# Algy/fast-slic

Measured on AMD Instinct MI355X. Metric: megapixels/sec @10 iters (1280x720 & 4K, K=1600); % HBM roofline, higher is better.
Workload: dtype u8/u16/i32 (integer SLIC); 1 GPU; 1280x720 RGB, K=1600, 10 iters (configs[1]), 8 frames/GPU; frames_per_gpu=8, global_frames=8, slots_per_gpu=6, submissions_per_launch_group=up to 2 (dynamic batching of the pipeline), inputs=device-resident uint8 RGB, device int16 labels, parallelism=frames sharded across GPUs, no collective

## Files before the change

### fast_slic_amd/_binding.py

```python
import ctypes as C
import os
import subprocess
import threading

import numpy as np

ARCH_NAME = "hip/gfx950"
_HERE = os.path.dirname(os.path.abspath(__file__))
_LIB_PATH = os.path.join(_HERE, "libfslic_hip.so")

CLUSTER_DTYPE = np.dtype([
    ("y", "<f4"), ("x", "<f4"), ("r", "<f4"), ("g", "<f4"), ("b", "<f4"), ("a", "<f4"),
    ("number", "<u2"), ("is_active", "u1"), ("is_updatable", "u1"), ("num_members", "<u4"),
])
assert CLUSTER_DTYPE.itemsize == 32

FSLIC_OK, FSLIC_E_INVALID, FSLIC_E_UNSUPPORTED, FSLIC_E_HIP, FSLIC_E_INTERNAL = range(5)


class Params(C.Structure):
    _fields_ = [
        ("max_iter", C.c_int32), ("compactness", C.c_float), ("min_size_factor", C.c_float),
        ("subsample_stride", C.c_int32), ("convert_to_lab", C.c_int32),
        ("manhattan_spatial_dist", C.c_int32), ("preemptive", C.c_int32),
        ("preemptive_thres", C.c_float), ("num_threads", C.c_int32), ("debug_mode", C.c_int32),
        ("abi", C.c_int32), ("variant", C.c_int32), ("reserved", C.c_int32 * 4),
    ]


EXPORTS = [
    "fslic_hip_device_count", "fslic_hip_create", "fslic_hip_destroy", "fslic_hip_initialize_clusters",
    "fslic_hip_iterate", "fslic_hip_iterate_device", "fslic_hip_iterate_batch", "fslic_hip_submit_group",
    "fslic_hip_wait_group", "fslic_hip_rgb_to_lab",
    "fslic_hip_enforce_connectivity", "fslic_hip_last_prelabels", "fslic_hip_last_timing_report",
    "fslic_hip_last_device_times", "fslic_hip_set_launch_timing", "fslic_hip_last_assign_loop", "fslic_hip_last_group_frames", "fslic_hip_last_path", "fslic_hip_last_launch_mode", "fslic_hip_group_done", "fslic_hip_last_error", "fslic_hip_version",
    "fslic_hip_get_connectivity", "fslic_hip_knn_connectivity", "fslic_hip_get_mask_density", "fslic_hip_cluster_density_to_mask",
    "fslic_hip_pipeline_submit", "fslic_hip_pipeline_drain", "fslic_hip_pipeline_batching", "fslic_hip_last_host_topk_frames",
    "fslic_hip_separate_pass_redos", "fslic_hip_copy_bandwidth", "fslic_hip_last_recorder_report",
    "fslic_hip_crf_new", "fslic_hip_crf_free", "fslic_hip_crf_copy", "fslic_hip_crf_get_params", "fslic_hip_crf_set_params",
    "fslic_hip_crf_set_compat", "fslic_hip_crf_get_compat", "fslic_hip_crf_num_classes", "fslic_hip_crf_first_time",
    "fslic_hip_crf_last_time", "fslic_hip_crf_num_frames", "fslic_hip_crf_pop_frame", "fslic_hip_crf_push_frame", "fslic_hip_crf_frame",
    "fslic_hip_crf_frame_time", "fslic_hip_crf_frame_set_clusters", "fslic_hip_crf_frame_get_clusters",
    "fslic_hip_crf_frame_set_connectivity", "fslic_hip_crf_frame_set_connectivity_csr", "fslic_hip_crf_frame_get_connectivity",
    "fslic_hip_crf_frame_set_mask", "fslic_hip_crf_frame_set_proba", "fslic_hip_crf_frame_set_unbiased", "fslic_hip_crf_frame_set_unary",
    "fslic_hip_crf_frame_get_unary", "fslic_hip_crf_frame_spatial_energy", "fslic_hip_crf_frame_temporal_energy",
    "fslic_hip_crf_frame_get_inferred", "fslic_hip_crf_frame_reset_inferred", "fslic_hip_crf_initialize", "fslic_hip_crf_inference",
    "fslic_hip_crf_expf_host", "fslic_hip_crf_expf_device",
    "fslic_hip_pool_workspace_size", "fslic_hip_pool", "fslic_hip_pool_finalize", "fslic_hip_unpool",
]

_lib = None
_lib_lock = threading.Lock()


def build_library(force=False):
    csrc = os.path.join(_HERE, "csrc")
    args = ["make", "-s", "-C", csrc]
    if force:
        args.append("-B")
    subprocess.check_call(args)
    return _LIB_PATH


def _preload_torch_hip_runtime():
    import importlib.util
    import sys
    if "torch" in sys.modules:
        return
    try:
        spec = importlib.util.find_spec("torch")
    except (ImportError, ValueError):
        spec = None
    if spec is None or not spec.origin:
        return
    cand = os.path.join(os.path.dirname(spec.origin), "lib", "libamdhip64.so")
    if os.path.exists(cand):
        try:
            C.CDLL(cand, mode=C.RTLD_GLOBAL)
        except OSError:
            pass


def load_library():
    global _lib
    with _lib_lock:
        if _lib is not None:
            return _lib
        _preload_torch_hip_runtime()
        if not os.path.exists(_LIB_PATH):
            raise ImportError(
                "fast_slic_amd: %s is missing; build it with `python -c 'import __graft_entry__ as g; g.build()'` "
                "or `make -C fast_slic_amd/csrc` (there is no CPU fallback)" % _LIB_PATH)
        lib = C.CDLL(os.environ.get("FSLIC_LIB") or _LIB_PATH)
        vp, i32 = C.c_void_p, C.c_int
        lib.fslic_hip_device_count.restype = i32
        lib.fslic_hip_create.argtypes = [i32, i32, C.POINTER(vp)]
        lib.fslic_hip_destroy.argtypes = [vp]
        lib.fslic_hip_destroy.restype = None
        lib.fslic_hip_initialize_clusters.argtypes = [i32, i32, i32, vp, vp]
        lib.fslic_hip_iterate.argtypes = [vp, C.POINTER(Params), i32, i32, i32, vp, vp, vp]
        lib.fslic_hip_iterate_device.argtypes = [vp, i32, C.POINTER(Params), i32, i32, i32, vp, vp, vp]
        lib.fslic_hip_iterate_batch.argtypes = [vp, C.POINTER(Params), i32, i32, i32, i32, vp, vp, vp, i32]
        lib.fslic_hip_submit_group.argtypes = [vp, i32, C.POINTER(Params), i32, i32, i32, i32, vp, vp, vp]
        lib.fslic_hip_wait_group.argtypes = [vp, i32]
        lib.fslic_hip_pipeline_submit.argtypes = [vp, C.POINTER(Params), i32, i32, i32, i32, vp, vp, vp]
        lib.fslic_hip_pipeline_drain.argtypes = [vp, C.POINTER(C.c_double), C.POINTER(C.c_longlong), C.POINTER(C.c_longlong), C.POINTER(C.c_longlong)]
        lib.fslic_hip_pipeline_batching.argtypes = [vp, i32]
        lib.fslic_hip_last_host_topk_frames.argtypes = [vp, i32]
        lib.fslic_hip_separate_pass_redos.argtypes = [vp, i32]
        if hasattr(lib, "fslic_hip_copy_bandwidth"):
            lib.fslic_hip_copy_bandwidth.argtypes = [vp, C.c_size_t, i32, C.POINTER(C.c_double)]
        lib.fslic_hip_group_done.argtypes = [vp, i32]
        lib.fslic_hip_rgb_to_lab.argtypes = [vp, i32, i32, vp, i32, vp]
        lib.fslic_hip_enforce_connectivity.argtypes = [vp, vp, i32, i32, i32, i32]
        lib.fslic_hip_last_prelabels.argtypes = [vp, i32, vp]
        lib.fslic_hip_last_timing_report.argtypes = [vp]
        lib.fslic_hip_last_timing_report.restype = C.c_char_p
        if hasattr(lib, "fslic_hip_last_recorder_report"):
            lib.fslic_hip_last_recorder_report.argtypes = [vp, C.POINTER(C.c_char_p), C.POINTER(C.c_size_t)]
        lib.fslic_hip_last_device_times.argtypes = [vp, i32, C.POINTER(C.c_float), C.POINTER(C.c_float)]
        lib.fslic_hip_set_launch_timing.argtypes = [vp, i32]
        lib.fslic_hip_last_assign_loop.argtypes = [vp, i32, C.POINTER(C.c_float), C.POINTER(C.c_double), C.POINTER(C.c_int)]
        lib.fslic_hip_last_group_frames.argtypes = [vp, i32]
        lib.fslic_hip_last_path.argtypes = [vp, i32]
        lib.fslic_hip_last_launch_mode.argtypes = [vp, i32]
        if hasattr(lib, "fslic_hip_lab_force_generic"):
            lib.fslic_hip_lab_force_generic.argtypes = [vp, i32]
        lib.fslic_hip_last_error.restype = C.c_char_p
        lib.fslic_hip_version.restype = C.c_char_p
        lib.fslic_hip_get_connectivity.argtypes = [vp, i32, i32, i32, vp, vp, vp]
        lib.fslic_hip_knn_connectivity.argtypes = [i32, i32, i32, vp, C.c_size_t, vp, vp]
        lib.fslic_hip_get_mask_density.argtypes = [vp, i32, i32, i32, vp, vp, vp, vp]
        lib.fslic_hip_cluster_density_to_mask.argtypes = [vp, i32, i32, i32, vp, vp, vp]
        if hasattr(lib, "fslic_hip_crf_new"):
            _declare_crf(lib)
        if hasattr(lib, "fslic_hip_pool"):
            _declare_pool(lib)
        _lib = lib
        return lib


def _declare_crf(lib):
    vp, i32, sz, f32 = C.c_void_p, C.c_int, C.c_size_t, C.c_float
    for name, args in [
        ("new", [sz, sz, C.POINTER(vp)]), ("copy", [vp, C.POINTER(vp)]), ("get_params", [vp, vp]), ("set_params", [vp, vp]),
        ("set_compat", [vp, i32, f32]), ("get_compat", [vp, i32, C.POINTER(f32)]), ("num_classes", [vp, C.POINTER(sz), C.POINTER(sz)]),
        ("first_time", [vp]), ("last_time", [vp]), ("pop_frame", [vp]), ("push_frame", [vp, C.POINTER(vp)]),
        ("frame", [vp, i32, C.POINTER(vp)]), ("frame_time", [vp]), ("frame_set_clusters", [vp, vp]), ("frame_get_clusters", [vp, vp]),
        ("frame_set_connectivity", [vp, i32, vp, vp, sz]), ("frame_set_connectivity_csr", [vp, i32, vp, vp]),
        ("frame_get_connectivity", [vp, vp, vp]), ("frame_set_mask", [vp, vp, f32]), ("frame_set_proba", [vp, vp]),
        ("frame_set_unbiased", [vp]), ("frame_set_unary", [vp, vp]), ("frame_get_unary", [vp, vp]),
        ("frame_spatial_energy", [vp, i32, i32, C.POINTER(f32)]), ("frame_temporal_energy", [vp, vp, i32, C.POINTER(f32)]),
        ("frame_get_inferred", [vp, vp]), ("frame_reset_inferred", [vp]), ("initialize", [vp]), ("inference", [vp, vp, sz]),
        ("expf_host", [vp, vp, sz, i32]), ("expf_device", [vp, vp, vp, sz]),
    ]:
        f = getattr(lib, "fslic_hip_crf_" + name)
        f.argtypes = args
        f.restype = i32
    lib.fslic_hip_crf_free.argtypes = [vp]
    lib.fslic_hip_crf_free.restype = None
    lib.fslic_hip_crf_num_frames.argtypes = [vp]
    lib.fslic_hip_crf_num_frames.restype = sz


def _declare_pool(lib):
    vp, i32 = C.c_void_p, C.c_int
    lib.fslic_hip_pool_workspace_size.argtypes = [i32, i32, i32, i32, C.POINTER(C.c_size_t)]
# ... 3 lines not shown
    for name in ("pool_workspace_size", "pool", "pool_finalize", "unpool"):
        getattr(lib, "fslic_hip_" + name).restype = i32


def _raise(rc):
    msg = load_library().fslic_hip_last_error().decode("utf-8", "replace")
    if rc == FSLIC_E_INVALID:
        raise ValueError(msg)
    if rc == FSLIC_E_UNSUPPORTED:
        raise NotImplementedError(msg)
    raise RuntimeError(msg)


def _check(rc):
    if rc != FSLIC_OK:
        _raise(rc)


class Engine(object):

    def __init__(self, device=0, n_slots=1):
        lib = load_library()
        h = C.c_void_p()
        _check(lib.fslic_hip_create(int(device), int(n_slots), C.byref(h)))
        self._h = h
        self.device = int(device)
        self.n_slots = int(n_slots)

    def close(self):
        if getattr(self, "_h", None):
            load_library().fslic_hip_destroy(self._h)
            self._h = None

    def __del__(self):
        try:
            self.close()
        except Exception:
            pass

    def rgb_to_lab(self, image, convert=True):
        image = np.ascontiguousarray(image, dtype=np.uint8)
        H, W, ch = image.shape
        if ch != 3:
            raise ValueError("nchan != 3")
        out = np.empty((H, W, 4), np.uint8)
        _check(load_library().fslic_hip_rgb_to_lab(self._h, H, W, image.ctypes.data, int(bool(convert)), out.ctypes.data))
        return out

    def enforce_connectivity(self, labels_u16, K, min_threshold):
        out = np.ascontiguousarray(labels_u16, dtype=np.uint16).copy()
        H, W = out.shape
        _check(load_library().fslic_hip_enforce_connectivity(self._h, out.ctypes.data, H, W, int(K), int(min_threshold)))
        return out

    @staticmethod
    def _plane(a, dtype):
        if isinstance(a, (int, np.integer)):
            return C.c_void_p(int(a)), None
        arr = np.ascontiguousarray(a, dtype=dtype)
        return C.c_void_p(arr.ctypes.data), arr

    def get_connectivity(self, labels, H, W, K):
        ptr, keep = self._plane(labels, np.uint16)
        num = np.zeros(K, np.int32)
        nb = np.zeros((K, 12), np.uint32)
        _check(load_library().fslic_hip_get_connectivity(self._h, H, W, int(K), ptr, num.ctypes.data, nb.ctypes.data))
        return num, nb

    def get_mask_density(self, clusters, labels, mask, H, W):
        lp, k1 = self._plane(labels, np.uint16)
        mp, k2 = self._plane(mask, np.uint8)
        cl = np.ascontiguousarray(clusters)
        dens = np.zeros(cl.shape[0], np.uint8)
        _check(load_library().fslic_hip_get_mask_density(self._h, H, W, cl.shape[0], cl.ctypes.data, lp, mp, dens.ctypes.data))
        return dens

    def cluster_density_to_mask(self, labels, densities, H, W, out=None):
        lp, k1 = self._plane(labels, np.uint16)
        d = np.ascontiguousarray(densities, dtype=np.uint8)
        if out is None:
            res = np.empty((H, W), np.uint8)
            op = C.c_void_p(res.ctypes.data)
        else:
            res, op = out, C.c_void_p(int(out))
        _check(load_library().fslic_hip_cluster_density_to_mask(self._h, H, W, d.shape[0], lp, d.ctypes.data, op))
        return res

    def iterate(self, image, clusters, params):
        H, W, _ = image.shape
        labels = np.empty((H, W), np.uint16)
        _check(load_library().fslic_hip_iterate(self._h, C.byref(params), H, W, clusters.shape[0],
                                                image.ctypes.data, clusters.ctypes.data, labels.ctypes.data))
        return labels

    def iterate_device(self, d_rgb_ptr, d_labels_ptr, H, W, clusters, params, slot=0):
        _check(load_library().fslic_hip_iterate_device(self._h, int(slot), C.byref(params), H, W, clusters.shape[0],
                                                       C.c_void_p(d_rgb_ptr), clusters.ctypes.data, C.c_void_p(d_labels_ptr)))

    def iterate_batch(self, rgb_ptrs, cluster_arrays, label_ptrs, H, W, params, device_ptrs):
        n = len(rgb_ptrs)
        K = cluster_arrays[0].shape[0]
        PA = C.c_void_p * n
        a_rgb = PA(*[C.c_void_p(int(p)) for p in rgb_ptrs])
        a_cl = PA(*[C.c_void_p(c.ctypes.data) for c in cluster_arrays])
        a_lab = PA(*[C.c_void_p(int(p)) for p in label_ptrs])
        _check(load_library().fslic_hip_iterate_batch(self._h, C.byref(params), H, W, K, n,
# ... 315 lines not shown
```

### fast_slic_amd/csrc/cca.hip

```cpp
#include "device_common.h"

namespace fslic {

constexpr uint32_t kNoAdopt = 0xFFFFFFFFu;
static __device__ __forceinline__ uint32_t* n_parent(const CcaDev& c, uint32_t n) { return reinterpret_cast<uint32_t*>(c.nrec + n); }
static __device__ __forceinline__ uint32_t n_leader(const CcaDev& c, uint32_t n) { return reinterpret_cast<const uint32_t*>(c.nrec + n)[1]; }
static __device__ __forceinline__ uint32_t n_local(const CcaDev& c, uint32_t n) { return reinterpret_cast<const uint32_t*>(c.nrec + n)[2]; }
static __device__ __forceinline__ uint32_t n_adopt(const CcaDev& c, uint32_t n) { return reinterpret_cast<const uint32_t*>(c.nrec + n)[3]; }

static __device__ __forceinline__ uint32_t lds_ld(uint32_t* p) {
    return __hip_atomic_load(p, __ATOMIC_RELAXED, __HIP_MEMORY_SCOPE_WORKGROUP);
}
static __device__ __forceinline__ void lds_st(uint32_t* p, uint32_t v) {
    __hip_atomic_store(p, v, __ATOMIC_RELAXED, __HIP_MEMORY_SCOPE_WORKGROUP);
}
static __device__ __forceinline__ uint32_t lds_find(uint32_t* par, uint32_t x) {
    for (;;) {
        const uint32_t p = lds_ld(par + x);
        if (p == x) return x;
        const uint32_t gp = lds_ld(par + p);
        if (gp == p) return p;
        lds_st(par + x, gp);
        x = gp;
    }
// ... 6 lines not shown
        if (a < b) { const uint32_t t = a; a = b; b = t; }
        const uint32_t old = atomicMin(par + a, b);
        if (old == a) return;
        a = old;
    }
}

static __device__ __forceinline__ uint32_t lds_find_ro(uint32_t* par, uint32_t x) {
    uint32_t p = lds_ld(par + x);
    while (p != x) { x = p; p = lds_ld(par + x); }
    return x;
}

typedef unsigned long long u64;
static __device__ __forceinline__ uint32_t lane_left0(uint32_t v) { return (uint32_t)__builtin_amdgcn_update_dpp(0, (int)v, 0x138 , 0xF, 0xF, true); }
static __device__ __forceinline__ uint32_t lane_left_or(uint32_t old, uint32_t v) { return (uint32_t)__builtin_amdgcn_update_dpp((int)old, (int)v, 0x138, 0xF, 0xF, false); }
static __device__ __forceinline__ uint32_t rank_in(u64 m) { return __builtin_amdgcn_mbcnt_hi((uint32_t)(m >> 32), __builtin_amdgcn_mbcnt_lo((uint32_t)m, 0u)); }
static __device__ __forceinline__ uint32_t* lds_at(uint32_t* base, uint32_t off) { return reinterpret_cast<uint32_t*>(reinterpret_cast<char*>(base) + off); }
static __device__ __forceinline__ void ldsb_union(uint32_t* par, uint32_t a, uint32_t b) {
    for (;;) {
        for (;;) {
            const uint32_t pa = lds_ld(lds_at(par, a)), pb = lds_ld(lds_at(par, b));
            if (pa == a && pb == b) break;
            a = pa; b = pb;
        }
        if (a == b) return;
        if (a < b) { const uint32_t t = a; a = b; b = t; }
        const uint32_t old = atomicMin(lds_at(par, a), b);
        if (old == a) return;
        a = old;
    }
}

#if defined(FSLIC_LAB) && FSLIC_LAB == 2
#define LOC_STAMP(i_) do { __syncthreads(); if (threadIdx.x == 0) c.cand_leader[(size_t)c.N - 8 * (size_t)(blockIdx.z * gridDim.y + blockIdx.y + 1) + (i_)] = (int32_t)((uint32_t)__builtin_amdgcn_s_memrealtime() - loc_t); } while (0)
#else
#define LOC_STAMP(i_) do { } while (0)
#endif
__global__ __launch_bounds__(256) __attribute__((amdgpu_num_sgpr(80))) void k_cca_local(CcaDev c) {
    const int tile_x = (int)blockIdx.y, tile_y = (int)blockIdx.z;
    c.select((int)blockIdx.x);
#if defined(FSLIC_LAB) && FSLIC_LAB == 2
    const uint32_t loc_t = (uint32_t)__builtin_amdgcn_s_memrealtime();
    if (threadIdx.x == 0) c.cand_leader[(size_t)c.N - 8 * (size_t)(blockIdx.z * gridDim.y + blockIdx.y + 1) + 7] = (int32_t)loc_t;
#endif
    constexpr int T = kCcaTile;
    constexpr int TH = kCcaTileH;
    constexpr int RW = TH / 4;
    static_assert(T == 64 && RW == 8, "lane = column, eight rows per wavefront");
    __shared__ uint32_t s_last[4][T];
    __shared__ uint32_t s_par[T * TH];
    __shared__ uint32_t s_area[T * TH];
    __shared__ uint32_t s_nroots, s_base;
    if (threadIdx.x == 0) s_nroots = 0;
    const int lane = LANE();
    const int wave = (int)rfl((uint32_t)(threadIdx.x >> 6));
    const int tx0 = tile_x * T, ty0 = tile_y * TH;
    const int ly0 = wave * RW;
    const int ncols = min(c.W - tx0, T), nrows = min(max(c.H - (ty0 + ly0), 0), RW);
    const u64 colmask = ncols >= 64 ? ~0ull : ((1ull << ncols) - 1ull);
#define ROW_MASK(i_) ((i_) < nrows ? colmask : 0ull)

    const uint16_t* const rowp = c.in + ((size_t)(ty0 + ly0) * c.W + tx0);
    uint32_t lbl[RW];
#pragma unroll
    for (int i = 0; i < RW; ++i) {
        lbl[i] = 0x10000u | (uint32_t)((i & 1) << 6) | (uint32_t)lane;
        if (lanes(ROW_MASK(i))) lbl[i] = (uint32_t)rowp[(size_t)i * c.W + lane];
    }
    LOC_STAMP(0);
    uint32_t nodev[RW];
    uint32_t up_root = 0, pend_a = 0, pend_b = 0;
    u64 pending = 0;
    auto run_pending = [&]() {
#if !(FSLIC_EXP & 128)
        if (lanes(pending)) ldsb_union(s_par, pend_a, pend_b);
#endif
        pending = 0;
    };
#pragma unroll
    for (int i = 0; i < RW; ++i) {
        const uint32_t l = lbl[i];
        const u64 m = ballot(l != lane_left0(l)) | 1ull;
        const uint32_t node = ((uint32_t)(ly0 + i) << 8) + (rank_in(m >> 1) << 2);
        nodev[i] = node;
        if (lanes(m)) { *lds_at(s_par, node) = node; *lds_at(s_area, node) = 0u; }
        if (i == RW - 1) s_last[wave][lane] = l | (node << 17);
        uint32_t cur_root = node;
        if (i > 0) {
            const u64 same = ballot(lbl[i - 1] == l);
            const u64 other = ballot(lane_left0(up_root) != up_root);
            const u64 rep = same & (m | other | ~(same << 1));
#if !(FSLIC_EXP & 64)
            if (lanes(rep)) __hip_atomic_fetch_min(lds_at(s_par, node), up_root, __ATOMIC_RELAXED, __HIP_MEMORY_SCOPE_WORKGROUP);
            cur_root = lds_ld(lds_at(s_par, node));
#endif
            const u64 need = rep & ballot(up_root != cur_root);
            if (need & pending) run_pending();
            const bool nd = lanes(need);
            pend_a = nd ? up_root : pend_a;
            pend_b = nd ? cur_root : pend_b;
            pending |= need;
        }
        up_root = cur_root;
    }
    run_pending();
    lds_barrier();
    LOC_STAMP(1);
    if (wave > 0) {
        const uint32_t l = lbl[0];
        const uint32_t prev = s_last[wave - 1][lane];
        const u64 m = ballot(l != lane_left0(l)) | 1ull;
        const u64 same = ballot((prev & 0x1FFFFu) == l);
        const u64 first = same & (m | ~(same << 1));
#if !(FSLIC_EXP & 128)
        if (lanes(first)) ldsb_union(s_par, nodev[0], prev >> 17);
#endif
    }
    lds_barrier();
    LOC_STAMP(2);
    uint32_t root[RW];
#pragma unroll
    for (int i = 0; i < RW; ++i) root[i] = lds_ld(lds_at(s_par, nodev[i]));
#pragma unroll
    for (int i = 0; i < RW; ++i) root[i] = lds_ld(lds_at(s_par, root[i]));
    for (;;) {
        uint32_t nx[RW];
#pragma unroll
        for (int i = 0; i < RW; ++i) nx[i] = lds_ld(lds_at(s_par, root[i]));
        u64 moved = 0;
#pragma unroll
        for (int i = 0; i < RW; ++i) { moved |= ballot(nx[i] != root[i]); root[i] = nx[i]; }
        if (!moved) break;
    }
    uint32_t pos[RW];
    uint32_t wcount = 0;
    const uint32_t lane_p1 = (uint32_t)lane + 1u;
#pragma unroll
    for (int i = 0; i < RW; ++i) {
        const u64 ok = ROW_MASK(i);
        const uint32_t l = lbl[i];
        const u64 m = ballot(l != lane_left0(l)) | 1ull;
        const u64 e = (m >> 1) | (1ull << 63);
        const uint32_t len_part = (lanes(e) ? lane_p1 : 0u) - (lanes(m) ? (uint32_t)lane : 0u);
#if !(FSLIC_EXP & 512)
        if (lanes((m | e) & ok)) atomicAdd(lds_at(s_area, root[i]), len_part);
#endif
        const u64 mr = m & ok & ballot(root[i] == nodev[i]);
        pos[i] = lanes(mr) ? wcount + rank_in(mr) : 0xFFFFFFFFu;
        wcount += (uint32_t)__popcll(mr);
    }
    LOC_STAMP(3);
    uint32_t wbase = 0;
    if (wcount != 0u && lanes(1ull)) {
        asm volatile("ds_add_rtn_u32 %0, %1, %2\n\ts_waitcnt lgkmcnt(0)" : "=v"(wbase) : "v"((uint32_t)(size_t)(__attribute__((address_space(3))) uint32_t*)&s_nroots), "v"(wcount) : "memory");
    }
    wbase = rfl(wbase);
    lds_barrier();
    LOC_STAMP(4);
    if (wave == 0 && lanes(1ull)) {
        const uint32_t nr = lds_ld(&s_nroots);
        uint32_t base = 0;
        if (nr) asm volatile("global_atomic_add %0, %1, %2, off sc0\n\ts_waitcnt vmcnt(0)" : "=v"(base) : "v"(c.counters), "v"(nr) : "memory");
        lds_st(&s_base, base);
    }
#pragma unroll
    for (int i = 0; i < RW; ++i)
        if (pos[i] != 0xFFFFFFFFu) lds_st(lds_at(s_par, root[i]), wbase + pos[i]);
    lds_barrier();
    LOC_STAMP(5);
    const uint32_t nbase = (uint32_t)(tile_y * (int)gridDim.y + tile_x) * (uint32_t)kCcaTilePx;
    const uint32_t gbase = s_base + wbase;
    uint32_t ar[RW];
#pragma unroll
    for (int i = 0; i < RW; ++i) ar[i] = lds_ld(lds_at(s_area, root[i]));
    wave_lds_sync();
    uint32_t* const stage = s_area + ly0 * T;
    uint32_t* const s_edge = &s_last[wave][lane ? 1 : 0];
    const __amdgpu_buffer_rsrc_t lr = __builtin_amdgcn_make_buffer_rsrc(c.lid, 0, (int)((uint32_t)c.N * 2u), 0x00020000);
    uint32_t up_id = 0xFFFu;
#pragma unroll
    for (int i = 0; i < RW; ++i) {
        const uint32_t y = (uint32_t)(ty0 + ly0 + i);
        const uint32_t id = lds_ld(lds_at(s_par, root[i]));
        const uint32_t left_id = lane_left_or(tile_x == 0 ? up_id : 0xFFFu, id);
        if (lanes(ROW_MASK(i))) __builtin_amdgcn_raw_buffer_store_b16((uint16_t)id, lr, lane * 2, (int)((y * (uint32_t)c.W + (uint32_t)tx0) * 2u), 16 );
        if (lanes(0x8000000000000001ull)) lds_st(s_edge + 2 * i, lbl[i] | (id << 16));
        if (pos[i] != 0xFFFFFFFFu) lds_st(stage + pos[i], (uint32_t)(i * T + lane) | ((ar[i] - 1u) << 9) | (left_id << 20));
        up_id = id;
    }
    wave_lds_sync();
    const uint32_t n0 = nbase + wbase;
    const uint32_t first_px = (uint32_t)(ty0 + ly0) * (uint32_t)c.W + (uint32_t)tx0;
    for (uint32_t j = (uint32_t)lane; j < wcount; j += 64u) {
        const uint32_t w = lds_ld(stage + j);
        const uint32_t n = n0 + j, a = ((w >> 9) & 0x7FFu) + 1u, ad = w >> 20;
        c.nrec[n] = make_uint4(n, first_px + __umul24((w >> 6) & 7u, (uint32_t)c.W) + (w & 63u), a, ad == 0xFFFu ? kNoAdopt : nbase + ad);
        c.narea[n] = a;
        c.roots[gbase + j] = n;
    }
    if (lane < 2 * RW) (c.vedge + (size_t)(nbase / (uint32_t)kCcaTilePx) * (2 * TH))[2 * ly0 + lane] = lds_ld(&s_last[wave][lane]);
    LOC_STAMP(6);
#undef ROW_MASK
}

static __device__ __forceinline__ uint32_t g_load(uint32_t* p) {
    return __hip_atomic_load(p, __ATOMIC_RELAXED, __HIP_MEMORY_SCOPE_AGENT);
}
static __device__ __forceinline__ uint32_t node_at(const CcaDev& c, int y, int x, size_t p) {
    return (uint32_t)((y / kCcaTileH) * c.tiles_x + x / kCcaTile) * (uint32_t)kCcaTilePx + (uint32_t)c.lid[p];
}
static __device__ __forceinline__ uint32_t node_of(const CcaDev& c, uint32_t p) {
    const int y = (int)(p / (uint32_t)c.W);
    return node_at(c, y, (int)(p - (uint32_t)y * (uint32_t)c.W), p);
}
static __device__ __forceinline__ uint32_t g_find(const CcaDev& c, uint32_t x) {
    for (;;) {
        const uint32_t p = g_load(n_parent(c, x));
        if (p == x) return x;
        const uint32_t gp = g_load(n_parent(c, p));
        if (gp == p) return p;
        __hip_atomic_store(n_parent(c, x), gp, __ATOMIC_RELAXED, __HIP_MEMORY_SCOPE_AGENT);
        x = gp;
    }
}
static __device__ __forceinline__ void g_union(const CcaDev& c, uint32_t a, uint32_t b) {
    for (;;) {
        a = g_find(c, a);
        b = g_find(c, b);
        if (a == b) return;
        if (n_leader(c, a) < n_leader(c, b)) { const uint32_t t = a; a = b; b = t; }
        if (atomicCAS(n_parent(c, a), a, b) == a) return;
    }
}

static __device__ __forceinline__ uint2 g_load2(const CcaDev& c, uint32_t n) {
    const unsigned long long v = __hip_atomic_load(reinterpret_cast<unsigned long long*>(c.nrec + n), __ATOMIC_RELAXED, __HIP_MEMORY_SCOPE_AGENT);
    return make_uint2((uint32_t)v, (uint32_t)(v >> 32));
}
static __device__ __forceinline__ uint32_t g_find_leader(const CcaDev& c, uint32_t& x, uint2 r) {
    for (;;) {
// ... 484 lines not shown
                return;
            }
            tie_heap_select(c, M, (uint32_t)K, astar, s_area, s_lead, s_key, s_bcnt, s_bstart, s_bfill, s_w);
            if (tid == 0) c.counters[3] = 0u;
            return;
        }
    }
    int bsh = 0;
    while ((((uint32_t)c.N - 1u) >> bsh) >= (uint32_t)kSelBuckets) bsh++;
    for (int i = tid; i < 3 * kSelBuckets; i += 1024) s_bcnt[i] = 0;
    __syncthreads();
    for (uint32_t i = tid; i < M; i += 1024)
        if (s_area[i] >= astar) atomicAdd(&s_bcnt[s_lead[i] >> bsh], 1u);
    __syncthreads();
    {
        const uint32_t a = s_bcnt[2 * tid], b = s_bcnt[2 * tid + 1];
        uint32_t n_keep;
        const uint32_t ex = block_excl_scan_1024(a + b, s_w, n_keep);
        s_bstart[2 * tid] = ex;
        s_bstart[2 * tid + 1] = ex + a;
    }
    __syncthreads();
    for (uint32_t i = tid; i < M; i += 1024)
        if (s_area[i] >= astar) {
            const uint32_t b = s_lead[i] >> bsh;
            s_key[s_bstart[b] + atomicAdd(&s_bfill[b], 1u)] = s_lead[i];
        }
    __syncthreads();
    for (uint32_t i0 = tid; i0 < M; i0 += 4096) {
        uint32_t me[4], r[4], nd[4];
        bool kept[4];
#pragma unroll
        for (int u = 0; u < 4; ++u) nd[u] = c.cand_area[min(i0 + 1024u * u, M - 1u)];
#pragma unroll
        for (int u = 0; u < 4; ++u) {
            const uint32_t i = i0 + 1024u * u;
            kept[u] = i < M && s_area[i] >= astar;
            me[u] = kept[u] ? s_lead[i] : 0u;
            r[u] = 0u;
            if (kept[u]) {
                const uint32_t b = me[u] >> bsh;
                const uint32_t lo = s_bstart[b], hi = lo + s_bcnt[b];
                r[u] = lo;
                for (uint32_t j = lo; j < hi; ++j) r[u] += (uint32_t)(s_key[j] < me[u]);
            }
        }
#pragma unroll
        for (int u = 0; u < 4; ++u) if (kept[u]) c.nfinal[nd[u]] = (uint16_t)r[u];
    }
    if (tid == 0) c.counters[3] = 0u;
}

static int root_pass_blocks(const CcaDev& c) {
    const int b = (c.N / 12 + 255) / 256;
    return b < 1 ? 1 : b;
}

void launch_cca_phase1(const CcaDev& c, int nframes, hipStream_t st) {
    constexpr int T = kCcaTile;
    const int tx = (c.W + T - 1) / T, ty = (c.H + kCcaTileH - 1) / kCcaTileH;
    launch(k_cca_local, dim3(nframes, tx, ty), dim3(256), 0, st, c);
    const int nh = (ty - 1) * ((c.W + kSeamPx - 1) / kSeamPx), nv = (tx - 1) * ((c.H + kSeamPx - 1) / kSeamPx);
    if (nh + nv > 0)
        launch(k_cca_border, dim3((nh + nv + 255) / 256, nframes), dim3(256), 0, st, c, nh, nv);
    launch(k_cca_compress, dim3(root_pass_blocks(c) * nframes), dim3(256), 0, st, c, nframes);
}

void launch_cca_select(const CcaDev& c, int nframes, hipStream_t st) {
    long long need = (long long)c.N / (c.min_threshold > 1 ? c.min_threshold : 1) + 1;
    int cap = 1024;
    while (cap < need && cap < kSelCap) cap <<= 1;
    if (cap > kSelCap) cap = kSelCap;
    const size_t lds = (3 * (size_t)cap + 3 * (size_t)kSelBuckets) * sizeof(uint32_t);
    static_assert(kSelBins <= 3 * kSelBuckets, "the selection histogram reuses the ranking buckets");
    static std::atomic<int> attr_state[64];
    if (!max_dynamic_lds_on_this_device(k_cca_select, (int)((3 * (size_t)kSelCap + 3 * (size_t)kSelBuckets) * sizeof(uint32_t)), attr_state)) {
        while (cap > 1024 && (3 * (size_t)cap + 3 * (size_t)kSelBuckets) * sizeof(uint32_t) > 64 * 1024) cap >>= 1;
        const size_t lds_small = (3 * (size_t)cap + 3 * (size_t)kSelBuckets) * sizeof(uint32_t);
        launch(k_cca_select, dim3(nframes), dim3(1024), lds_small, st, c, cap);
        return;
    }
    launch(k_cca_select, dim3(nframes), dim3(1024), lds, st, c, cap);
}

__global__ __launch_bounds__(256) void k_cca_reset_final(CcaDev c) {
    const uint32_t n = c.counters[0];
    for (uint32_t i = blockIdx.x * blockDim.x + threadIdx.x; i < n; i += gridDim.x * blockDim.x) {
        const uint32_t r = c.roots[i];
        if (*n_parent(c, r) == r) c.nfinal[r] = 0xFFFFu;
    }
}
__global__ void k_cca_set_kept(CcaDev c, const int32_t* __restrict__ leaders, const uint16_t* __restrict__ labels, int n) {
    const int i = blockIdx.x * blockDim.x + threadIdx.x;
    if (i < n) c.nfinal[node_of(c, (uint32_t)leaders[i])] = labels[i];
}
__global__ void k_cca_gather_area(CcaDev c) {
    const uint32_t M = c.counters[1];
    for (uint32_t i = blockIdx.x * blockDim.x + threadIdx.x; i < M; i += gridDim.x * blockDim.x) c.cand_area[i] = c.narea[node_of(c, (uint32_t)c.cand_leader[i])];
}
void launch_cca_gather_area(const CcaDev& c, hipStream_t st) {
    launch(k_cca_gather_area, dim3(64), dim3(256), 0, st, c);
}

void launch_cca_set_kept(const CcaDev& c, const int32_t* d_leaders, const uint16_t* d_labels, int n, hipStream_t st) {
    launch(k_cca_reset_final, dim3(root_pass_blocks(c)), dim3(256), 0, st, c);
    if (n <= 0) return;
    launch(k_cca_set_kept, dim3((n + 255) / 256), dim3(256), 0, st, c, d_leaders, d_labels, n);
// ... 124 lines not shown
```

### fast_slic_amd/csrc/host_utils.cpp

```cpp
#include "engine_internal.h"

#include <algorithm>
#include <cmath>
#include <cstring>

using namespace fslic;

extern "C" {

int fslic_hip_initialize_clusters(int H, int W, int K, const uint8_t* rgb, fslic_cluster* cl) {
    if (!rgb || !cl) return fail(FSLIC_E_INVALID, "NULL pointer argument");
    if (H <= 0 || W <= 0 || K <= 0) return FSLIC_OK;
    const int n_y = (int)sqrt((double)K);
    std::vector<int> n_xs(n_y, K / n_y);
    int remainder = K % n_y, row = 0;
    while (remainder-- > 0) {
        n_xs[row]++;
        row += 2;
        if (row >= n_y) row = 1 % n_y;
    }
    const int h = (H + n_y - 1) / n_y;
    int acc = 0;
    for (int i = 0; i < H; i += h) {
        const int w = (W + n_xs[std::min(i / h, n_y - 1)] - 1) / n_xs[std::min(i / h, n_y - 1)];
// ... 2 lines not shown
            cl[acc].y = (float)clampi(i + h / 2, 0, H - 1);
            cl[acc].x = (float)clampi(j + w / 2, 0, W - 1);
            cl[acc].is_active = 1;
            cl[acc].is_updatable = 1;
            acc++;
        }
    }
    for (; acc < K; acc++) {
        cl[acc].is_active = 1;
        cl[acc].is_updatable = 1;
        cl[acc].y = (float)(H / 2);
        cl[acc].x = (float)(W / 2);
    }
    for (int k = 0; k < K; k++) {
        const size_t base = (size_t)W * (int)cl[k].y + (int)cl[k].x;
        cl[k].r = rgb[3 * base];
        cl[k].g = rgb[3 * base + 1];
        cl[k].b = rgb[3 * base + 2];
        cl[k].number = (uint16_t)k;
        cl[k].num_members = 0;
    }
    return FSLIC_OK;
}

int fslic_hip_rgb_to_lab(fslic_engine* e, int H, int W, const uint8_t* rgb, int convert, uint8_t* lab4) {
    if (!e || !rgb || !lab4) return fail(FSLIC_E_INVALID, "NULL pointer argument");
    if (H <= 0 || W <= 0 || (long long)H * W >= (1ll << 31)) return fail(FSLIC_E_INVALID, "bad image size");
    HIPCHK(hipSetDevice(e->device));
    const size_t N = (size_t)H * W;
    uint8_t* d_rgb = nullptr;
    uint32_t* d_lab = nullptr;
    HIPCHK(hipMalloc((void**)&d_rgb, N * 3));
    if (hipMalloc((void**)&d_lab, N * 4) != hipSuccess) { hipFree(d_rgb); return fail(FSLIC_E_HIP, "hipMalloc failed"); }
    SlotLease lease(e);
    if (lease.take() != FSLIC_OK) { hipFree(d_rgb); hipFree(d_lab); return FSLIC_E_INVALID; }
    Slot& sl = e->slots[lease.slot];
    hipStream_t st = sl.st;
    hipMemcpyAsync(d_rgb, rgb, N * 3, hipMemcpyHostToDevice, st);
    FrameDev f{};
    f.N = (int)N; f.H = H; f.W = W;
    f.lab = d_lab;
    const uint8_t* in1[1] = {d_rgb};
    if (upload_ptrs(sl, 1, in1, nullptr) != FSLIC_OK) { hipFree(d_rgb); hipFree(d_lab); return FSLIC_E_HIP; }
    f.rgbs = reinterpret_cast<const uint8_t* const*>(sl.d_ptrs);
    launch_rgb_to_lab(f, 1, convert, e->tables, false, st);
    hipMemcpyAsync(lab4, d_lab, N * 4, hipMemcpyDeviceToHost, st);
    hipError_t err = hipStreamSynchronize(st);
    hipFree(d_rgb);
    hipFree(d_lab);
    if (err != hipSuccess) return fail(FSLIC_E_HIP, hipGetErrorString(err));
    return FSLIC_OK;
}

int fslic_hip_enforce_connectivity(fslic_engine* e, uint16_t* labels, int H, int W, int K, int min_threshold) {
    if (!e || !labels) return fail(FSLIC_E_INVALID, "NULL pointer argument");
    if (H <= 0 || W <= 0 || (long long)H * W >= (1ll << 31)) return fail(FSLIC_E_INVALID, "bad image size");
    if (K <= 0) return FSLIC_OK;
    if (K > 65536) return fail(FSLIC_E_INVALID, "K must be at most 65536 (labels are uint16)");
    HIPCHK(hipSetDevice(e->device));
    SlotLease lease(e);
    int rc = lease.take();
    if (rc) return rc;
    Slot& s = e->slots[lease.slot];
    int S = (int)sqrt((double)H * W / K);
    if (S < 1) S = 1;
    HIPCHK(hipStreamSynchronize(s.st));
    rc = prepare(e, s, H, W, K, S, 1);
    if (rc) return rc;
    s.keyH = s.keyW = s.keyK = 0;
    s.have_pre = false;
    const size_t N = (size_t)H * W;
    HIPCHK(hipMemsetAsync(s.zero_block, 0, s.zero_bytes, s.st));
    HIPCHK(hipMemcpyAsync(s.d_out_stage, labels, N * 2, hipMemcpyHostToDevice, s.st));
    uint16_t* outs[1] = {s.d_out_stage};
    rc = upload_ptrs(s, 1, nullptr, outs);
    if (rc) return rc;
    const CcaDev c = cca_view(s, 0, s.d_out_stage, 0, K, min_threshold);
    cca_enqueue(s, c, 0, 1);
    HIPCHK(hipMemcpyAsync(s.h_misc, s.d_misc, 64, hipMemcpyDeviceToHost, s.st));
    HIPCHK(hipStreamSynchronize(s.st));
    rc = cca_finish_group(s, 0, 1, s.d_out_stage, 0, K, min_threshold);
    if (rc) return rc;
    HIPCHK(hipMemcpyAsync(labels, s.d_out_stage, N * 2, hipMemcpyDeviceToHost, s.st));
    HIPCHK(hipStreamSynchronize(s.st));
    return FSLIC_OK;
}

namespace {
struct Staged {
    void* p = nullptr;
    bool owned = false;
    ~Staged() { if (owned && p) hipFree(p); }
};
bool is_device_pointer(const void* p) {
    hipPointerAttribute_t a;
    if (hipPointerGetAttributes(&a, p) != hipSuccess) { (void)hipGetLastError(); return false; }
    return a.type == hipMemoryTypeDevice;
}
int stage_in(const void* src, size_t bytes, hipStream_t st, Staged& out) {
    if (is_device_pointer(src)) { out.p = const_cast<void*>(src); return FSLIC_OK; }
    HIPCHK(hipMalloc(&out.p, std::max<size_t>(bytes, 16)));
    out.owned = true;
    HIPCHK(hipMemcpyAsync(out.p, src, bytes, hipMemcpyHostToDevice, st));
    return FSLIC_OK;
}
int device_scratch(size_t bytes, Staged& out) {
    HIPCHK(hipMalloc(&out.p, std::max<size_t>(bytes, 16)));
    out.owned = true;
    return FSLIC_OK;
}
int check_map(const fslic_engine* e, int H, int W, int K) {
    if (!e) return fail(FSLIC_E_INVALID, "NULL engine");
    if (H <= 0 || W <= 0 || (long long)H * W >= (1ll << 31)) return fail(FSLIC_E_INVALID, "bad image size");
    if (K <= 0 || K > 65536) return fail(FSLIC_E_INVALID, "K must be in [1, 65536]");
    return FSLIC_OK;
}
}

int fslic_hip_get_mask_density(fslic_engine* e, int H, int W, int K, const fslic_cluster* clusters, const uint16_t* labels,
                               const uint8_t* mask, uint8_t* densities) {
    int rc = check_map(e, H, W, K);
    if (rc) return rc;
    if (!clusters || !labels || !mask || !densities) return fail(FSLIC_E_INVALID, "NULL pointer argument");
    HIPCHK(hipSetDevice(e->device));
    SlotLease lease(e);
    if ((rc = lease.take())) return rc;
    hipStream_t st = e->slots[lease.slot].st;
    const size_t N = (size_t)H * W;
    Staged d_lab, d_mask, d_sums;
    if ((rc = stage_in(labels, N * 2, st, d_lab)) || (rc = stage_in(mask, N, st, d_mask)) || (rc = device_scratch((size_t)K * 4, d_sums))) return rc;
    HIPCHK(hipMemsetAsync(d_sums.p, 0, (size_t)K * 4, st));
    launch_mask_sums((const uint16_t*)d_lab.p, (const uint8_t*)d_mask.p, (uint32_t*)d_sums.p, H, W, K, st);
    std::vector<uint32_t> sums((size_t)K);
    HIPCHK(hipMemcpyAsync(sums.data(), d_sums.p, (size_t)K * 4, hipMemcpyDeviceToHost, st));
    HIPCHK(hipStreamSynchronize(st));
    for (int k = 0; k < K; k++) {
        const uint32_t q = sums[(size_t)k] / std::max<uint32_t>(clusters[k].num_members, 1u);
        densities[k] = (uint8_t)std::min<int>(255, (int)q);
// ... 147 lines not shown
```

### include/fslic_hip.h

```cpp
#ifndef FSLIC_HIP_H
#define FSLIC_HIP_H

#include <stddef.h>
#include <stdint.h>

#ifdef __cplusplus
extern "C" {
#endif

#define FSLIC_HIP_ARCH_NAME "hip/gfx950"

enum {
    FSLIC_OK = 0,
    FSLIC_E_INVALID = 1,
    FSLIC_E_UNSUPPORTED = 2,
    FSLIC_E_HIP = 3,
    FSLIC_E_INTERNAL = 4
};

typedef struct fslic_cluster {
    float y, x, r, g, b, a;
    uint16_t number;
    uint8_t is_active;
    uint8_t is_updatable;
// ... 9 lines not shown
    int32_t manhattan_spatial_dist;
    int32_t preemptive;
    float preemptive_thres;
    int32_t num_threads;
    int32_t debug_mode;
    int32_t abi;
    int32_t variant;
    int32_t reserved[4];
} fslic_params;
#define FSLIC_PARAMS_ABI 0x46533033

enum {
    FSLIC_VARIANT_SLIC = 0,
    FSLIC_VARIANT_LSC = 1,
    FSLIC_VARIANT_REALDIST = 2,
    FSLIC_VARIANT_REALDIST_L2 = 3,
    FSLIC_VARIANT_REALDIST_NOQ = 4
};

typedef struct fslic_engine fslic_engine;

int fslic_hip_device_count(void);

int fslic_hip_create(int device, int n_slots, fslic_engine** out);
void fslic_hip_destroy(fslic_engine* e);

int fslic_hip_initialize_clusters(int H, int W, int K, const uint8_t* rgb, fslic_cluster* clusters);

int fslic_hip_iterate(fslic_engine* e, const fslic_params* p, int H, int W, int K,
                      const uint8_t* rgb, fslic_cluster* clusters, uint16_t* labels);

int fslic_hip_iterate_device(fslic_engine* e, int slot, const fslic_params* p, int H, int W, int K,
                             const uint8_t* d_rgb, fslic_cluster* clusters, uint16_t* d_labels);

int fslic_hip_iterate_batch(fslic_engine* e, const fslic_params* p, int H, int W, int K, int n_frames,
                            const uint8_t* const* rgb, fslic_cluster* const* clusters,
                            uint16_t* const* labels, int device_ptrs);

int fslic_hip_submit_group(fslic_engine* e, int slot, const fslic_params* p, int H, int W, int K, int n_frames,
                           const uint8_t* const* d_rgb, fslic_cluster* const* clusters, uint16_t* const* d_labels);
int fslic_hip_wait_group(fslic_engine* e, int slot);
int fslic_hip_group_done(fslic_engine* e, int slot);

int fslic_hip_pipeline_submit(fslic_engine* e, const fslic_params* p, int H, int W, int K, int n_frames,
                              const uint8_t* const* d_rgb, fslic_cluster* const* clusters, uint16_t* const* d_labels);
int fslic_hip_pipeline_drain(fslic_engine* e, double* device_ms, long long* groups, long long* frames,
                             long long* host_topk_frames);
int fslic_hip_pipeline_batching(fslic_engine* e, int max_frames_per_group);


int fslic_hip_rgb_to_lab(fslic_engine* e, int H, int W, const uint8_t* rgb, int convert, uint8_t* lab4);

int fslic_hip_enforce_connectivity(fslic_engine* e, uint16_t* labels, int H, int W, int K, int min_threshold);


int fslic_hip_get_connectivity(fslic_engine* e, int H, int W, int K, const uint16_t* labels,
                               int* num_neighbors, uint32_t* neighbors);

int fslic_hip_knn_connectivity(int H, int W, int K, const fslic_cluster* clusters, size_t n_neighbors,
                               int* num_neighbors, uint32_t* neighbors);

int fslic_hip_get_mask_density(fslic_engine* e, int H, int W, int K, const fslic_cluster* clusters,
                               const uint16_t* labels, const uint8_t* mask, uint8_t* densities);

int fslic_hip_cluster_density_to_mask(fslic_engine* e, int H, int W, int K, const uint16_t* labels,
                                      const uint8_t* densities, uint8_t* result);

int fslic_hip_last_prelabels(fslic_engine* e, int slot, uint16_t* prelabels);

const char* fslic_hip_last_timing_report(fslic_engine* e);

int fslic_hip_last_recorder_report(fslic_engine* e, const char** report, size_t* length);

int fslic_hip_last_device_times(fslic_engine* e, int slot, float* total_ms, float* full_assign_ms);

int fslic_hip_set_launch_timing(fslic_engine* e, int on);
int fslic_hip_last_assign_loop(fslic_engine* e, int slot, float* sum_ms, double* visited_px, int* launches);

int fslic_hip_last_group_frames(fslic_engine* e, int slot);

int fslic_hip_last_launch_mode(fslic_engine* e, int slot);

int fslic_hip_last_path(fslic_engine* e, int slot);

int fslic_hip_last_host_topk_frames(fslic_engine* e, int slot);

int fslic_hip_separate_pass_redos(fslic_engine* e, int slot);

int fslic_hip_copy_bandwidth(fslic_engine* e, size_t bytes, int reps, double* gb_per_s);

typedef struct fslic_crf fslic_crf;
typedef struct fslic_crf_frame fslic_crf_frame;
typedef struct fslic_crf_params {
    float spatial_w, temporal_w, spatial_srgb, temporal_srgb, spatial_sxy, spatial_smooth_w, spatial_smooth_sxy;
} fslic_crf_params;

int fslic_hip_crf_new(size_t num_classes, size_t num_nodes, fslic_crf** out);
void fslic_hip_crf_free(fslic_crf* crf);
int fslic_hip_crf_copy(fslic_crf* crf, fslic_crf** out);
int fslic_hip_crf_get_params(fslic_crf* crf, fslic_crf_params* out);
int fslic_hip_crf_set_params(fslic_crf* crf, const fslic_crf_params* params);
int fslic_hip_crf_set_compat(fslic_crf* crf, int cls, float compat_value);
int fslic_hip_crf_get_compat(fslic_crf* crf, int cls, float* out);
int fslic_hip_crf_num_classes(fslic_crf* crf, size_t* num_classes, size_t* num_nodes);
int fslic_hip_crf_first_time(fslic_crf* crf);
int fslic_hip_crf_last_time(fslic_crf* crf);
// ... 43 lines not shown
```

Baseline: 61170 megapixels/sec.

## Merge tile-interior small components in CCA tile pass to shrink node graph

The tile-local connected-component kernel now detects components whose area is below the minimum threshold and that do not touch an open tile border, and merges them into a left or upper neighbour inside the tile instead of emitting them as global nodes. Border-touching components get a large area bias so they are never dropped locally. The goal is fewer global nodes for the later root and merge passes, and the root-pass grid is shrunk to match. In exchange the kernel gains an extra barrier, an LDS pointer-chasing loop and flag encoding in s_par. A new API that returns the node count is added for inspection.

```diff
diff --git a/fast_slic_amd/_binding.py b/fast_slic_amd/_binding.py
--- a/fast_slic_amd/_binding.py
+++ b/fast_slic_amd/_binding.py
@@ -32,7 +32,7 @@
     "fslic_hip_device_count", "fslic_hip_create", "fslic_hip_destroy", "fslic_hip_initialize_clusters",
     "fslic_hip_iterate", "fslic_hip_iterate_device", "fslic_hip_iterate_batch", "fslic_hip_submit_group",
     "fslic_hip_wait_group", "fslic_hip_rgb_to_lab",
-    "fslic_hip_enforce_connectivity", "fslic_hip_last_prelabels", "fslic_hip_last_timing_report",
+    "fslic_hip_enforce_connectivity", "fslic_hip_enforce_connectivity_nodes", "fslic_hip_last_prelabels", "fslic_hip_last_timing_report",
     "fslic_hip_last_device_times", "fslic_hip_set_launch_timing", "fslic_hip_last_assign_loop", "fslic_hip_last_group_frames", "fslic_hip_last_path", "fslic_hip_last_launch_mode", "fslic_hip_group_done", "fslic_hip_last_error", "fslic_hip_version",
     "fslic_hip_get_connectivity", "fslic_hip_knn_connectivity", "fslic_hip_get_mask_density", "fslic_hip_cluster_density_to_mask",
     "fslic_hip_pipeline_submit", "fslic_hip_pipeline_drain", "fslic_hip_pipeline_batching", "fslic_hip_last_host_topk_frames",
@@ -113,6 +113,8 @@
         lib.fslic_hip_group_done.argtypes = [vp, i32]
         lib.fslic_hip_rgb_to_lab.argtypes = [vp, i32, i32, vp, i32, vp]
         lib.fslic_hip_enforce_connectivity.argtypes = [vp, vp, i32, i32, i32, i32]
+        if hasattr(lib, "fslic_hip_enforce_connectivity_nodes"):
+            lib.fslic_hip_enforce_connectivity_nodes.argtypes = [vp, vp, i32, i32, i32, i32, C.POINTER(C.c_uint32)]
         lib.fslic_hip_last_prelabels.argtypes = [vp, i32, vp]
         lib.fslic_hip_last_timing_report.argtypes = [vp]
         lib.fslic_hip_last_timing_report.restype = C.c_char_p
@@ -222,6 +224,13 @@
         H, W = out.shape
         _check(load_library().fslic_hip_enforce_connectivity(self._h, out.ctypes.data, H, W, int(K), int(min_threshold)))
         return out
+
+    def enforce_connectivity_nodes(self, labels_u16, K, min_threshold):
+        out = np.ascontiguousarray(labels_u16, dtype=np.uint16).copy()
+        H, W = out.shape
+        n = C.c_uint32(0)
+        _check(load_library().fslic_hip_enforce_connectivity_nodes(self._h, out.ctypes.data, H, W, int(K), int(min_threshold), C.byref(n)))
+        return out, int(n.value)
 
     @staticmethod
     def _plane(a, dtype):
diff --git a/fast_slic_amd/csrc/cca.hip b/fast_slic_amd/csrc/cca.hip
--- a/fast_slic_amd/csrc/cca.hip
+++ b/fast_slic_amd/csrc/cca.hip
@@ -82,6 +82,7 @@
     __shared__ uint32_t s_par[T * TH];
     __shared__ uint32_t s_area[T * TH];
     __shared__ uint32_t s_nroots, s_base;
+    __shared__ uint32_t s_up0[4];
     if (threadIdx.x == 0) s_nroots = 0;
     const int lane = LANE();
     const int wave = (int)rfl((uint32_t)(threadIdx.x >> 6));
@@ -163,22 +164,43 @@
         for (int i = 0; i < RW; ++i) { moved |= ballot(nx[i] != root[i]); root[i] = nx[i]; }
         if (!moved) break;
     }
-    uint32_t pos[RW];
-    uint32_t wcount = 0;
-    const uint32_t lane_p1 = (uint32_t)lane + 1u;
+    const uint32_t thr_c = (uint32_t)min(max(c.min_threshold, 0), 0x10000);
+    const bool may_drop = thr_c > 1u;
+    const bool open_l = may_drop && tile_x > 0, open_r = may_drop && tile_x + 1 < (int)gridDim.y;
+    const bool open_t = may_drop && wave == 0 && tile_y > 0, open_b = may_drop && wave == 3 && tile_y + 1 < (int)gridDim.z;
+    const uint32_t lane_p1 = (uint32_t)lane + 1u + ((open_r && lane == 63) ? 0x10000u : 0u);
+    const uint32_t lane_m = (uint32_t)lane - ((open_l && lane == 0) ? 0x10000u : 0u);
 #pragma unroll
     for (int i = 0; i < RW; ++i) {
         const u64 ok = ROW_MASK(i);
         const uint32_t l = lbl[i];
         const u64 m = ballot(l != lane_left0(l)) | 1ull;
         const u64 e = (m >> 1) | (1ull << 63);
-        const uint32_t len_part = (lanes(e) ? lane_p1 : 0u) - (lanes(m) ? (uint32_t)lane : 0u);
+        uint32_t len_part = (lanes(e) ? lane_p1 : 0u) - (lanes(m) ? lane_m : 0u);
+        if ((i == 0 && open_t) || (i == RW - 1 && open_b)) len_part += lanes(m) ? 0x10000u : 0u;
 #if !(FSLIC_EXP & 512)
         if (lanes((m | e) & ok)) atomicAdd(lds_at(s_area, root[i]), len_part);
 #endif
-        const u64 mr = m & ok & ballot(root[i] == nodev[i]);
-        pos[i] = lanes(mr) ? wcount + rank_in(mr) : 0xFFFFFFFFu;
-        wcount += (uint32_t)__popcll(mr);
+    }
+    uint32_t ar[RW];
+    if (may_drop) {
+        if (lanes(1ull)) lds_st(&s_up0[wave], root[RW - 1]);
+        lds_barrier();
+#pragma unroll
+        for (int i = 0; i < RW; ++i) ar[i] = lds_ld(lds_at(s_area, root[i]));
+    }
+    uint32_t pos[RW];
+    uint32_t wcount = 0;
+#pragma unroll
+    for (int i = 0; i < RW; ++i) {
+        const uint32_t l = lbl[i];
+        const u64 m = ballot(l != lane_left0(l)) | 1ull;
+        const u64 mr = m & ROW_MASK(i) & ballot(root[i] == nodev[i]);
+        u64 dr = 0;
+        if (may_drop) dr = mr & ballot(ar[i] < thr_c) & ~((wave == 0 && i == 0) ? 1ull : 0ull);
+        const u64 mk = mr & ~dr;
+        pos[i] = lanes(mk) ? wcount + rank_in(mk) : (lanes(dr) ? 0xFFFFFFFEu : 0xFFFFFFFFu);
+        wcount += (uint32_t)__popcll(mk);
     }
     LOC_STAMP(3);
     uint32_t wbase = 0;
@@ -194,16 +216,44 @@
         if (nr) asm volatile("global_atomic_add %0, %1, %2, off sc0\n\ts_waitcnt vmcnt(0)" : "=v"(base) : "v"(c.counters), "v"(nr) : "memory");
         lds_st(&s_base, base);
     }
-#pragma unroll
-    for (int i = 0; i < RW; ++i)
-        if (pos[i] != 0xFFFFFFFFu) lds_st(lds_at(s_par, root[i]), wbase + pos[i]);
+    const uint32_t wflag = wbase | (may_drop ? 0x80000000u : 0u);
+    uint32_t up0 = 0;
+    if (may_drop && wave > 0) up0 = lds_ld(&s_up0[wave - 1]);
+#pragma unroll
+    for (int i = 0; i < RW; ++i) {
+        if (pos[i] < 0xFFFFFFFEu) lds_st(lds_at(s_par, root[i]), wflag + pos[i]);
+        if (may_drop) {
+            const uint32_t nb = lane_left_or(i == 0 ? up0 : root[i > 0 ? i - 1 : 0], root[i]);
+            if (pos[i] == 0xFFFFFFFEu) lds_st(lds_at(s_par, root[i]), nb);
+        }
+    }
     lds_barrier();
     LOC_STAMP(5);
+    uint32_t idv[RW];
+#pragma unroll
+    for (int i = 0; i < RW; ++i) idv[i] = lds_ld(lds_at(s_par, root[i]));
+    if (may_drop) {
+        if (ncols < T || nrows < RW) {
+#pragma unroll
+            for (int i = 0; i < RW; ++i) idv[i] = lanes(ROW_MASK(i)) ? idv[i] : 0x80000000u;
+        }
+        for (;;) {
+            u64 walking = 0;
+#pragma unroll
+            for (int i = 0; i < RW; ++i) {
+                const u64 un = ballot((int32_t)idv[i] >= 0);
+                walking |= un;
+                if (lanes(un)) idv[i] = lds_ld(lds_at(s_par, idv[i]));
+            }
+            if (!walking) break;
+        }
+    }
     const uint32_t nbase = (uint32_t)(tile_y * (int)gridDim.y + tile_x) * (uint32_t)kCcaTilePx;
     const uint32_t gbase = s_base + wbase;
-    uint32_t ar[RW];
-#pragma unroll
-    for (int i = 0; i < RW; ++i) ar[i] = lds_ld(lds_at(s_area, root[i]));
+    if (!may_drop) {
+#pragma unroll
+        for (int i = 0; i < RW; ++i) ar[i] = lds_ld(lds_at(s_area, root[i]));
+    }
     wave_lds_sync();
     uint32_t* const stage = s_area + ly0 * T;
     uint32_t* const s_edge = &s_last[wave][lane ? 1 : 0];
@@ -212,11 +262,11 @@
 #pragma unroll
     for (int i = 0; i < RW; ++i) {
         const uint32_t y = (uint32_t)(ty0 + ly0 + i);
-        const uint32_t id = lds_ld(lds_at(s_par, root[i]));
+        const uint32_t id = idv[i];
         const uint32_t left_id = lane_left_or(tile_x == 0 ? up_id : 0xFFFu, id);
         if (lanes(ROW_MASK(i))) __builtin_amdgcn_raw_buffer_store_b16((uint16_t)id, lr, lane * 2, (int)((y * (uint32_t)c.W + (uint32_t)tx0) * 2u), 16 );
         if (lanes(0x8000000000000001ull)) lds_st(s_edge + 2 * i, lbl[i] | (id << 16));
-        if (pos[i] != 0xFFFFFFFFu) lds_st(stage + pos[i], (uint32_t)(i * T + lane) | ((ar[i] - 1u) << 9) | (left_id << 20));
+        if (pos[i] < 0xFFFFFFFEu) lds_st(stage + pos[i], (uint32_t)(i * T + lane) | (((ar[i] & 0xFFFFu) - 1u) << 9) | (left_id << 20));
         up_id = id;
     }
     wave_lds_sync();
@@ -807,7 +857,7 @@
 }
 
 static int root_pass_blocks(const CcaDev& c) {
-    const int b = (c.N / 12 + 255) / 256;
+    const int b = (c.N / 48 + 255) / 256;
     return b < 1 ? 1 : b;
 }
 
diff --git a/fast_slic_amd/csrc/host_utils.cpp b/fast_slic_amd/csrc/host_utils.cpp
--- a/fast_slic_amd/csrc/host_utils.cpp
+++ b/fast_slic_amd/csrc/host_utils.cpp
@@ -78,7 +78,8 @@
     return FSLIC_OK;
 }
 
-int fslic_hip_enforce_connectivity(fslic_engine* e, uint16_t* labels, int H, int W, int K, int min_threshold) {
+static int enforce_connectivity_impl(fslic_engine* e, uint16_t* labels, int H, int W, int K, int min_threshold, uint32_t* n_nodes) {
+    if (n_nodes) *n_nodes = 0;
     if (!e || !labels) return fail(FSLIC_E_INVALID, "NULL pointer argument");
     if (H <= 0 || W <= 0 || (long long)H * W >= (1ll << 31)) return fail(FSLIC_E_INVALID, "bad image size");
     if (K <= 0) return FSLIC_OK;
@@ -105,11 +106,20 @@
     cca_enqueue(s, c, 0, 1);
     HIPCHK(hipMemcpyAsync(s.h_misc, s.d_misc, 64, hipMemcpyDeviceToHost, s.st));
     HIPCHK(hipStreamSynchronize(s.st));
+    if (n_nodes) *n_nodes = s.h_misc[4];
     rc = cca_finish_group(s, 0, 1, s.d_out_stage, 0, K, min_threshold);
     if (rc) return rc;
     HIPCHK(hipMemcpyAsync(labels, s.d_out_stage, N * 2, hipMemcpyDeviceToHost, s.st));
     HIPCHK(hipStreamSynchronize(s.st));
     return FSLIC_OK;
+}
+
+int fslic_hip_enforce_connectivity(fslic_engine* e, uint16_t* labels, int H, int W, int K, int min_threshold) {
+    return enforce_connectivity_impl(e, labels, H, W, K, min_threshold, nullptr);
+}
+int fslic_hip_enforce_connectivity_nodes(fslic_engine* e, uint16_t* labels, int H, int W, int K, int min_threshold, uint32_t* n_nodes) {
+    if (!n_nodes) return fail(FSLIC_E_INVALID, "NULL pointer argument");
+    return enforce_connectivity_impl(e, labels, H, W, K, min_threshold, n_nodes);
 }
 
 namespace {
diff --git a/include/fslic_hip.h b/include/fslic_hip.h
--- a/include/fslic_hip.h
+++ b/include/fslic_hip.h
@@ -85,6 +85,7 @@
 int fslic_hip_rgb_to_lab(fslic_engine* e, int H, int W, const uint8_t* rgb, int convert, uint8_t* lab4);
 
 int fslic_hip_enforce_connectivity(fslic_engine* e, uint16_t* labels, int H, int W, int K, int min_threshold);
+int fslic_hip_enforce_connectivity_nodes(fslic_engine* e, uint16_t* labels, int H, int W, int K, int min_threshold, uint32_t* n_nodes);
 
 
 int fslic_hip_get_connectivity(fslic_engine* e, int H, int W, int K, const uint16_t* labels,
```

Result: faster. 64260 megapixels/sec, median of 6 (+5.1%).
